# pratyushkumar211/industrial_nnmpc_2021

Measured on AMD Instinct MI355X. Metric: condensed-QP solves/sec (CDU offline datagen), higher is better.
Workload: dtype f64; 1 GPU; cdu_offline_data: synthetic CDU-size plant (n=4480 vars, m=8960 box rows, n_aug=284), 100000 sampled x0 per GPU per step, whole sequences u* written out; batch_per_gpu=100000, total_batch=100000, method=auto, parallelism=dp1 (sharded samples, 1 RCCL gather of the first moves pe...

## Files before the change

### include/nnmpc.h

```cpp
#ifndef NNMPC_H
#define NNMPC_H
#include <stdint.h>
#ifdef __cplusplus
extern "C" {
#endif

#define NNMPC_OK 0
#define NNMPC_EINVAL (-1)
#define NNMPC_EHIP (-2)
#define NNMPC_ENOMEM (-3)
#define NNMPC_ENOTIMPL (-4)

#define NNMPC_HOST 0
#define NNMPC_DEVICE 1

#define NNMPC_ST_OPTIMAL 0
#define NNMPC_ST_MAXITER 1
#define NNMPC_ST_NUMERIC 2

typedef struct nnmpc_qp nnmpc_qp;
typedef struct nnmpc_nn nnmpc_nn;

typedef struct {
  int32_t max_batch;
// ... 76 lines not shown
                            int32_t* status, int32_t* iters, int32_t ptr_kind, int32_t out_kind);

int nnmpc_qp_set_inverse(nnmpc_qp* h, const double* Hinv, const double* Kunc);

int nnmpc_qp_set_farfield(nnmpc_qp* h, int32_t W, int32_t r, const double* U, const double* Vx, const double* Vl);
int nnmpc_qp_farfield_missing(nnmpc_qp* h, int32_t* W);

int nnmpc_qp_first_moves(const double* u, int64_t ldu, const double* us, int32_t B, int32_t nu, double* out);
int nnmpc_qp_dims(nnmpc_qp* h, int32_t* n, int32_t* nu, int32_t* n_aug);
int nnmpc_qp_set_profiling(nnmpc_qp* h, int32_t on);
int nnmpc_qp_get_stats(nnmpc_qp* h, nnmpc_qp_stats* out, int32_t reset);

int nnmpc_qp_debug_factor_solve(nnmpc_qp* h, int32_t B, const float* dvec, const float* mask,
                                const float* rhs, float* sol);
int nnmpc_qp_debug_factor_fail(nnmpc_qp* h, int32_t B, int32_t* fail);

int nnmpc_nn_create(nnmpc_nn** out, int32_t nlayers, const int32_t* dims,
                    const double* const* W, const double* const* b, int32_t nx, int32_t nu,
                    int32_t with_uprev, const double* xscale, const double* ulb,
                    const double* uub, int32_t use_bf16, int32_t max_batch);
#define NNMPC_NN_STRUCTURED 0
#define NNMPC_NN_UNSTD 1
#define NNMPC_NN_UNSTD_RELU 2
int nnmpc_nn_create_ex(nnmpc_nn** out, int32_t nlayers, const int32_t* dims,
                       const double* const* W, const double* const* b, int32_t nx, int32_t nu,
                       int32_t with_uprev, const double* xscale, const double* ulb,
                       const double* uub, int32_t use_bf16, int32_t max_batch, int32_t form);
int nnmpc_nn_destroy(nnmpc_nn* h);
int nnmpc_nn_forward(nnmpc_nn* h, int32_t B, const double* x, const double* uprev,
                     const double* xs, const double* us, double* u, int32_t ptr_kind);
// ... 136 lines not shown
```

### industrial_nnmpc_2021_amd/_lib.py

```python
import ctypes as C
import os

_HERE = os.path.dirname(os.path.abspath(__file__))
LIB_PATH = os.path.join(_HERE, "libnnmpc_hip.so")

HOST, DEVICE = 0, 1
ST_OPTIMAL, ST_MAXITER, ST_NUMERIC = 0, 1, 2
OUT_SEQUENCE, OUT_FIRST_MOVE = 0, 1
EINVAL, EHIP, ENOMEM, ENOTIMPL = -1, -2, -3, -4


class QpOpts(C.Structure):
    _fields_ = [("max_batch", C.c_int32), ("nb", C.c_int32), ("max_ipm_iters", C.c_int32),
                ("max_polish_rounds", C.c_int32), ("max_refine", C.c_int32),
                ("max_rounds", C.c_int32), ("sub_steps", C.c_int32), ("stale_max_changes", C.c_int32),
                ("stale_cg_limit", C.c_int32), ("method", C.c_int32), ("asm_max_active", C.c_int32),
                ("asm_max_rounds", C.c_int32), ("asm_f32_rounds", C.c_int32), ("seg_max", C.c_int32), ("asm_tail_batch", C.c_int32), ("asm_predict_iters", C.c_int32), ("asm_overlap", C.c_int32), ("ipm_tol", C.c_float), ("refine_tol", C.c_double),
                ("bound_tol", C.c_double)]


class QpStats(C.Structure):
    _fields_ = [("problems", C.c_int64), ("rounds", C.c_int64), ("factorizations", C.c_int64),
                ("ipm_iterations", C.c_int64), ("panel_launches", C.c_int64),
                ("panel_ms", C.c_double), ("diag_ms", C.c_double), ("trsv_ms", C.c_double),
# ... 16 lines not shown
class ClModel(C.Structure):
    _fields_ = [(k, C.c_int32) for k in ("nx", "nu", "ny", "nd", "nz")] + \
               [(k, C.c_void_p) for k in ("A", "B", "C", "Bp", "Aaug", "Baug", "Caug", "L", "tb", "Qb", "Qy", "q0", "Cd",
                                          "Eb", "Xb", "Xu", "Qaug", "Raug", "Maug", "ulb", "uub", "x0", "xhat0", "uprev0")]


class ClSlot(C.Structure):
    _fields_ = [("kind", C.c_int32), ("qp", C.c_void_p), ("nlayers", C.c_int32), ("dims", C.c_void_p), ("W", C.c_void_p),
                ("b", C.c_void_p), ("with_uprev", C.c_int32), ("xscale", C.c_void_p), ("Kaug", C.c_void_p)]


EXPORTS = ["nnmpc_last_error", "nnmpc_qp_create", "nnmpc_qp_destroy", "nnmpc_qp_solve_batch",
           "nnmpc_qp_solve_batch_warm", "nnmpc_qp_solve_batch_ex", "nnmpc_qp_set_inverse", "nnmpc_qp_dims",
           "nnmpc_qp_first_moves", "nnmpc_qp_set_farfield", "nnmpc_qp_farfield_missing",
           "nnmpc_qp_set_profiling", "nnmpc_qp_get_stats", "nnmpc_qp_debug_factor_solve", "nnmpc_qp_debug_factor_fail",
           "nnmpc_nn_create", "nnmpc_nn_create_ex", "nnmpc_nn_destroy", "nnmpc_nn_forward", "nnmpc_nn_last_ms", "nnmpc_nn_last_hidden_ms",
           "nnmpc_train_create", "nnmpc_train_destroy", "nnmpc_train_set_data", "nnmpc_train_grad", "nnmpc_train_step",
           "nnmpc_train_epoch", "nnmpc_train_eval", "nnmpc_train_get_weights", "nnmpc_train_set_weights",
           "nnmpc_train_snapshot", "nnmpc_train_restore", "nnmpc_train_last_ms", "nnmpc_train_dw_slices",
           "nnmpc_train_padding_max",
           "nnmpc_train_group_create", "nnmpc_train_group_destroy", "nnmpc_train_group_set_data",
           "nnmpc_train_group_epoch", "nnmpc_train_group_eval", "nnmpc_train_group_get_weights",
           "nnmpc_train_group_set_weights", "nnmpc_train_group_snapshot", "nnmpc_train_group_restore",
           "nnmpc_train_group_padding_max", "nnmpc_train_group_last_ms", "nnmpc_train_group_last_launches",
           "nnmpc_chain_create", "nnmpc_chain_destroy", "nnmpc_chain_run", "nnmpc_chain_reset", "nnmpc_chain_last_ms",
           "nnmpc_ts_create", "nnmpc_ts_destroy", "nnmpc_ts_solve_batch",
           "nnmpc_cl_create", "nnmpc_cl_destroy", "nnmpc_cl_run", "nnmpc_cl_reset", "nnmpc_cl_last_ms",
           "nnmpc_cl_set_plant", "nnmpc_cl_last_plant_ms", "nnmpc_cstrs_flow",
           "nnmpc_device_count", "nnmpc_set_device", "nnmpc_device_synchronize", "nnmpc_dev_mem_info",
           "nnmpc_dev_malloc", "nnmpc_dev_free", "nnmpc_dev_memset", "nnmpc_memcpy_h2d", "nnmpc_memcpy_d2h",
# ... 30 lines not shown
    lib.nnmpc_qp_solve_batch_warm.argtypes = [vp, i32, dp, dp, dp, dp, dp, dp, dp, dp, i32]
    lib.nnmpc_qp_set_inverse.restype = i32
    lib.nnmpc_qp_set_inverse.argtypes = [vp, dp, dp]
    lib.nnmpc_qp_set_farfield.restype = i32
    lib.nnmpc_qp_set_farfield.argtypes = [vp, i32, i32, dp, dp, dp]
    lib.nnmpc_qp_farfield_missing.restype = i32
    lib.nnmpc_qp_farfield_missing.argtypes = [vp, C.POINTER(i32)]
    lib.nnmpc_qp_set_profiling.restype = i32
    lib.nnmpc_qp_set_profiling.argtypes = [vp, i32]
    lib.nnmpc_qp_get_stats.restype = i32
    lib.nnmpc_qp_get_stats.argtypes = [vp, C.POINTER(QpStats), i32]
    lib.nnmpc_qp_debug_factor_solve.restype = i32
    lib.nnmpc_qp_debug_factor_solve.argtypes = [vp, i32, dp, dp, dp, dp]
    lib.nnmpc_qp_debug_factor_fail.restype = i32
    lib.nnmpc_qp_debug_factor_fail.argtypes = [vp, i32, dp]
    lib.nnmpc_nn_create.restype = i32
    lib.nnmpc_nn_create.argtypes = [C.POINTER(vp), i32, C.POINTER(i32), C.POINTER(dp), C.POINTER(dp),
                                    i32, i32, i32, dp, dp, dp, i32, i32]
    lib.nnmpc_nn_create_ex.restype = i32
    lib.nnmpc_nn_create_ex.argtypes = lib.nnmpc_nn_create.argtypes + [i32]
    lib.nnmpc_nn_destroy.restype = i32
    lib.nnmpc_nn_destroy.argtypes = [vp]
    lib.nnmpc_nn_forward.restype = i32
    lib.nnmpc_nn_forward.argtypes = [vp, i32, dp, dp, dp, dp, dp, i32]
    lib.nnmpc_nn_last_ms.restype = i32
    lib.nnmpc_nn_last_ms.argtypes = [vp, C.POINTER(C.c_double), C.POINTER(C.c_double)]
    lib.nnmpc_nn_last_hidden_ms.restype = i32
    lib.nnmpc_nn_last_hidden_ms.argtypes = [vp, C.POINTER(C.c_double), C.POINTER(C.c_int32)]
    f64, pf64, pi32, pdp = C.c_double, C.POINTER(C.c_double), C.POINTER(i32), C.POINTER(dp)
    lib.nnmpc_train_create.restype = i32
# ... 196 lines not shown
```

### industrial_nnmpc_2021_amd/csrc/qp_predict.h

```cpp
#pragma once
#include "qp_asm.h"

namespace nnmpc {

typedef __bf16 pbf16x8 __attribute__((ext_vector_type(8)));
typedef float pf32x4 __attribute__((ext_vector_type(4)));
typedef unsigned int pu32x4 __attribute__((ext_vector_type(4)));
typedef unsigned int pu32x2 __attribute__((ext_vector_type(2)));
typedef float pf32x2 __attribute__((ext_vector_type(2)));
typedef __bf16 pbf16x2 __attribute__((ext_vector_type(2)));
typedef _Float16 pf16x2 __attribute__((ext_vector_type(2)));

constexpr int PRED_NW = 8;
constexpr int PRED_MAXIT = 64;
template <int NT> struct PredCfg {
  static constexpr int W = 16 * NT * PRED_NW;
  static constexpr int KS = W / 32;
  static constexpr int LDY = W + 8;
};
constexpr int PRED_W = PredCfg<4>::W;
constexpr int PRED_W2 = PredCfg<8>::W;

struct PredArgs {
  const pu32x4* Hf;
  int iters;
  int* itsum;
  int fac10;
  int adaptive;
  float beta[PRED_MAXIT];
};

template <int NT, int PT> __host__ __device__ constexpr int pred_lds_bytes(int nu) {
  return 16 * PT * PredCfg<NT>::LDY * 2 + 2 * 16 * PT * (nu + 4) * 4 + 16;
}

template <int NT> __host__ __device__ constexpr size_t pred_frag_index(int jtg, int ks, int lane) {
  return (((size_t)(jtg / NT) * PredCfg<NT>::KS + ks) * NT + (jtg % NT)) * 64 + lane;
}

__device__ __forceinline__ unsigned pred_bf16(float x) {
  const unsigned u = __float_as_uint(x);
  return (u + 0x7fffu + ((u >> 16) & 1u)) >> 16;
}

template <int NT, int PT, bool NU4 = true>
__global__ __launch_bounds__(64 * PRED_NW, 2) void asm_predict_k(AsmDev d, PredArgs a) {
  extern __shared__ __attribute__((aligned(16))) unsigned char sm_raw[];
  constexpr int KS = PredCfg<NT>::KS, LDY = PredCfg<NT>::LDY, MR = 16 * PT;
  unsigned short* Y = reinterpret_cast<unsigned short*>(sm_raw);
  const int ldb = d.nu + 4;
  float* lbs = reinterpret_cast<float*>(Y + MR * LDY);
  float* ubs = lbs + MR * ldb;
  int* nviol = reinterpret_cast<int*>(ubs + MR * ldb);
  float* rsum = reinterpret_cast<float*>(nviol + 1);
  constexpr int NTH = 64 * PRED_NW;
  const int tid = threadIdx.x, lane = tid & 63, w = __builtin_amdgcn_readfirstlane(tid >> 6);
  const int li = lane & 15, lq = lane >> 4;
  const int p0 = blockIdx.x * MR;
  for (int i = tid; i < MR * d.nu; i += NTH) {
    const int r = i / d.nu, k = i - r * d.nu;
    const size_t p = (size_t)min(p0 + r, d.nseg - 1);
    lbs[r * ldb + k] = (float)d.lb[p * d.nu + k];
    ubs[r * ldb + k] = (float)d.ub[p * d.nu + k];
  }
  for (int i = tid; i < MR * LDY / 2; i += NTH) reinterpret_cast<unsigned*>(Y)[i] = 0u;
  if (tid == 0) { *nviol = 0; rsum[0] = 0.f; rsum[1] = 0.f; }
  unsigned sx[NT][PT][2], sm[NT][PT][2];
#pragma unroll
  for (int jt = 0; jt < NT; ++jt)
#pragma unroll
    for (int pt = 0; pt < PT; ++pt) {
      const size_t p = (size_t)min(p0 + 16 * pt + li, d.nseg - 1);
      const double* xr = d.xunc + p * d.np + 16 * (w * NT + jt) + 4 * lq;
#pragma unroll
      for (int h = 0; h < 2; ++h) {
        const pf32x2 xu = {fminf(fmaxf((float)xr[2 * h], -60000.f), 60000.f), fminf(fmaxf((float)xr[2 * h + 1], -60000.f), 60000.f)};
        sx[jt][pt][h] = __builtin_bit_cast(unsigned, __builtin_convertvector(xu, pf16x2));
        sm[jt][pt][h] = 0u;
      }
    }
  int kc0[NT];
#pragma unroll
  for (int jt = 0; jt < NT; ++jt) kc0[jt] = (16 * (w * NT + jt) + 4 * lq) % d.nu;
  const bool st_words = (d.n & 3) == 0;
  const bool per32 = 32 % d.nu == 0;
  __syncthreads();
  const __amdgpu_buffer_rsrc_t rH = __builtin_amdgcn_make_buffer_rsrc(const_cast<pu32x4*>(a.Hf), 0, PRED_NW * KS * NT * 1024, 0x00020000);
  const int l16 = lane * 16;
  const int hw0 = w * (KS * NT * 1024);
  auto hload = [&](int ksn, int jt) __attribute__((always_inline)) {
    return __builtin_bit_cast(pu32x4, __builtin_amdgcn_raw_buffer_load_b128(rH, l16 + jt * 1024, hw0 + ksn * (NT * 1024), 0));
  };
  int nit = a.iters;
  int kb = 0;
  for (int it = 0; it < nit; ++it) {
    if (tid == 0) rsum[it & 1] = 0.f;
    pf32x4 acc[NT][PT];
#pragma unroll
    for (int jt = 0; jt < NT; ++jt)
#pragma unroll
      for (int pt = 0; pt < PT; ++pt) acc[jt][pt] = pf32x4{0.f, 0.f, 0.f, 0.f};
#ifdef PRED_NO_MFMA
    if (false) {
#else
    if (it > 0) {
#endif
      constexpr int RD = 3;
      pu32x4 hb[RD][NT];
      asm_sfor<0, RD - 1>([&](auto bc) __attribute__((always_inline)) {
        constexpr int b = decltype(bc)::value;
#pragma unroll
        for (int jt = 0; jt < NT; ++jt) hb[b][jt] = hload(b, jt);
      });
      asm_sfor<0, KS>([&](auto kc) __attribute__((always_inline)) {
        constexpr int ks = decltype(kc)::value, b = ks % RD;
        if constexpr (ks + RD - 1 < KS) {
#pragma unroll
          for (int jt = 0; jt < NT; ++jt) hb[(ks + RD - 1) % RD][jt] = hload(ks + RD - 1, jt);
        }
        pu32x4 yf[PT];
#pragma unroll
        for (int pt = 0; pt < PT; ++pt) yf[pt] = *reinterpret_cast<const pu32x4*>(Y + (16 * pt + li) * LDY + 32 * ks + 8 * lq);
#pragma unroll
        for (int jt = 0; jt < NT; ++jt)
#pragma unroll
          for (int pt = 0; pt < PT; ++pt)
            acc[jt][pt] = __builtin_amdgcn_mfma_f32_16x16x32_bf16(__builtin_bit_cast(pbf16x8, hb[b][jt]), __builtin_bit_cast(pbf16x8, yf[pt]),
                                                                  acc[jt][pt], 0, 0, 0);
        __builtin_amdgcn_sched_barrier(0);
      });
    }
    __syncthreads();
    if (it > 0) kb = rsum[(it - 1) & 1] > 0.f ? 0 : kb + 1;
    const pf32x2 beta2 = {a.beta[kb], a.beta[kb]};
    pf32x2 rdot = {0.f, 0.f};
    int yo = li * LDY + 16 * NT * w + 4 * lq, bo = li * ldb;
    asm volatile("" : "+v"(yo), "+v"(bo));
    unsigned short* Yl = Y + yo;
    const float* lbl = lbs + bo;
    const float* ubl = ubs + bo;
    int nv0 = 0;
#pragma unroll
    for (int pt = 0; pt < PT; ++pt) {
      pf32x4 lb4[2], ub4[2];
#pragma unroll
      for (int jt = 0; jt < NT; ++jt) {
        if constexpr (NU4) {
          if (jt < 2 || !per32) {
            lb4[jt & 1] = *reinterpret_cast<const pf32x4*>(lbl + 16 * pt * ldb + kc0[jt]);
            ub4[jt & 1] = *reinterpret_cast<const pf32x4*>(ubl + 16 * pt * ldb + kc0[jt]);
          }
        } else {
#pragma unroll
          for (int r = 0; r < 4; ++r) {
            const int k = kc0[jt] + r, kk = k >= d.nu ? k - d.nu : k;
            lb4[jt & 1][r] = lbl[16 * pt * ldb + kk];
            ub4[jt & 1][r] = ubl[16 * pt * ldb + kk];
          }
        }
        unsigned short* yp = Yl + 16 * pt * LDY + 16 * jt;
        const pu32x2 yw = *reinterpret_cast<const pu32x2*>(yp);
        unsigned yb[2];
#pragma unroll
        for (int h = 0; h < 2; ++h) {
          const pf32x2 xu = __builtin_convertvector(__builtin_bit_cast(pf16x2, sx[jt][pt][h]), pf32x2);
          const unsigned mw = sm[jt][pt][h], ywd = yw[h];
          const pf32x2 nu = {__uint_as_float(mw << 16), __uint_as_float(mw & 0xffff0000u)};
          const pf32x2 y = {__uint_as_float(ywd << 16), __uint_as_float(ywd & 0xffff0000u)};
          const pf32x2 ac = {acc[jt][pt][2 * h], acc[jt][pt][2 * h + 1]};
#ifdef PRED_NO_EPI
          const pf32x2 wv = xu - ac;
#else
          const pf32x2 wv = y + (xu - ac);
#endif
          const pf32x2 cl = {__builtin_amdgcn_fmed3f(wv[0], lb4[jt & 1][2 * h], ub4[jt & 1][2 * h]),
                             __builtin_amdgcn_fmed3f(wv[1], lb4[jt & 1][2 * h + 1], ub4[jt & 1][2 * h + 1])};
          const pf32x2 nun = wv - cl;
          const pf32x2 dn = nun - nu;
          const pf32x2 yn = beta2 * dn + nun;
          rdot += (y - nun) * dn;
// ... 69 lines not shown
```

### industrial_nnmpc_2021_amd/csrc/qp_solver.hip

```cpp
#include <hip/hip_runtime.h>
#include <stdint.h>
#include <stdio.h>
#include <stdarg.h>
#include <string.h>
#include <vector>
#include <algorithm>
#include <cmath>
#include <cstdlib>
#include "../../include/nnmpc.h"
#define ASM_WG_TU (-1)
#include "chol_kernels.h"
#include "gemm_kernels.h"
#include "qp_asm.h"
#include "qp_wide.h"
#include "qp_small.h"
#include "qp_predict.h"
#include "common.h"
static constexpr int ASM_SMALL9_LDS_MAX = 100 * 1024;

using namespace nnmpc;

namespace {

enum { PH_INIT = 0, PH_IPM = 1, PH_POLISH = 2, PH_DONE = 3 };
// ... 613 lines not shown
  struct Far { int W, r, rp; double *U, *Vx, *Vl, *cu; int* kt; double ksum; double efar; };
  std::vector<Far> far;
  std::vector<int> far_missing;
  double p_inf = 0.0;
  double *asm_tnorm = nullptr, *asm_tslack = nullptr;
  struct AsmView {
    double *lam = nullptr, *xh = nullptr, *xhw = nullptr, *tnorm = nullptr, *tslack = nullptr;
    float *lam32 = nullptr, *xh32 = nullptr;
    int *rowprob = nullptr, *kblk = nullptr, *counters = nullptr;
    int rows = 0;
  };
  AsmView view[2];
  struct PredWin { pu32x4* Hf = nullptr; double L = 0.0; int W = 0; };
  PredWin pred[2];
  int* pred_cnt = nullptr;
  double* asm_work;
  int seg_max;
  double* x0_64;
  float* x0_32;
  double* q64_all;
  float* uunc_all;
  double *lb_d, *ub_d;
  double* in_stage;
  hipStream_t stream;
  hipStream_t stream2 = nullptr;
  hipStream_t stream3 = nullptr, stream4 = nullptr;
  int asm_tail_budget = 50000;
  hipEvent_t ev_fork = nullptr, ev_join = nullptr, ev_join3 = nullptr, ev_join4 = nullptr;
  hipEvent_t ev_wfork = nullptr, ev_wide = nullptr;
  int* pin_cnt = nullptr;
// ... 329 lines not shown
        if (force_w >= 0) wide = force_w;
        else {
          HIPCHK(hipMemsetAsync(h->pred_cnt, 0, 4, s));
          hipLaunchKernelGGL(asm_extent_k, dim3((nprob + 63) / 64), dim3(256), 0, s, a, PRED_W - PRED_W / 4, PRED_W, h->pred_cnt);
          HIPCHK(hipMemcpyAsync(h->pin_cnt, h->pred_cnt, 4, hipMemcpyDeviceToHost, s));
          HIPCHK(stream_sync(s));
          wide = h->pin_cnt[0] * 4 > nprob;
          h->pin_cnt[0] = 0;
        }
      }
      if (wide && Wx < PRED_W2) {
        EvScope es(h, 5, 2.0 * (PRED_W2 - Wx) * (double)h->ka * nprob);
        gemm64(h, h->asm_xunc + Wx, h->np, h->x0_64, h->ka, h->Kunc64 + (size_t)Wx * h->ka, h->ka, segp, PRED_W2 - Wx, h->ka);
        Wx = PRED_W2; a.Wx = Wx;
      }
      const bool nu4 = h->nu % 4 == 0;
      const int W = wide ? PRED_W2 : PRED_W, MR = (wide || !nu4) ? 32 : 64;
      pa.Hf = h->pred[wide].Hf;
      pred_flops_per_it = 2.0 * W * (double)W * MR;
      h->stats.asm_predict_launches += 1;
      EvScope es(h, 10, 0.0);
      if (wide) hipLaunchKernelGGL((asm_predict_k<8, 2>), dim3((nprob + 31) / 32), dim3(64 * PRED_NW), (pred_lds_bytes<8, 2>(h->nu)), s, a, pa);
      else if (nu4) hipLaunchKernelGGL((asm_predict_k<4, 4>), dim3((nprob + 63) / 64), dim3(64 * PRED_NW), (pred_lds_bytes<4, 4>(h->nu)), s, a, pa);
      else hipLaunchKernelGGL((asm_predict_k<4, 2, false>), dim3((nprob + 31) / 32), dim3(64 * PRED_NW), (pred_lds_bytes<4, 2>(h->nu)), s, a, pa);
      a.pred_w = W;
      { static const int pf = getenv("NNMPC_PRED_F64") ? atoi(getenv("NNMPC_PRED_F64")) : 0; a.pred_f64 = pf; }
    }
  }
  hipLaunchKernelGGL(asm_init_k, dim3((segp + 3) / 4), dim3(256), 0, s, a, segp);
  const int lds_big = (a.max_active + ASM_TS) * 8;
  int* cnt = h->pin_cnt;
  memset(cnt, 0, 2 * ASM_NCNT * sizeof(int));
  int rounds = 0;
  int kprev = 0;
  HIPCHK(hipMemsetAsync(h->asm_counters, 0, 2 * ASM_NCNT * sizeof(int), s));
  if (small) {
    EvScope es(h, 4, 0.0);
    static const int g0 = getenv("NNMPC_SMALL_GRACE") ? atoi(getenv("NNMPC_SMALL_GRACE")) : ASM_SM_GRACE;
    hipLaunchKernelGGL((asm_small_k<2, 3, 4>), dim3(nprob), dim3(64), asm_small_lds_bytes(2, h->n, h->nu), s, a, a.max_rounds, g0);
    hipLaunchKernelGGL((asm_small_k<7, 1, 8>), dim3(nprob), dim3(64), asm_small_lds_bytes(7, h->n, h->nu), s, a, a.max_rounds, g0);
// ... 601 lines not shown
}

int nnmpc_qp_destroy(nnmpc_qp* h) {
  if (!h) return NNMPC_OK;
  hipDeviceSynchronize();
  for (void* p : h->allocs) hipFree(p);
  for (auto& g : h->far) { hipFree(g.U); hipFree(g.Vx); hipFree(g.Vl); hipFree(g.cu); hipFree(g.kt); }
  for (auto& sc : h->sc) if (sc.p) hipFree(sc.p);
  for (hipEvent_t e : h->ev_pool) hipEventDestroy(e);
  if (h->ev_fork) hipEventDestroy(h->ev_fork);
  if (h->ev_join) hipEventDestroy(h->ev_join);
  if (h->ev_join3) hipEventDestroy(h->ev_join3);
  if (h->ev_join4) hipEventDestroy(h->ev_join4);
  if (h->ev_wfork) hipEventDestroy(h->ev_wfork);
  if (h->ev_wide) hipEventDestroy(h->ev_wide);
  if (h->pin_cnt) hipHostFree(h->pin_cnt);
  if (h->pin_st) hipHostFree(h->pin_st);
  if (h->stream2) hipStreamDestroy(h->stream2);
  if (h->stream3) hipStreamDestroy(h->stream3);
  if (h->stream4) hipStreamDestroy(h->stream4);
  if (h->stream) hipStreamDestroy(h->stream);
  delete h;
  return NNMPC_OK;
}

int nnmpc_qp_set_inverse(nnmpc_qp* h, const double* Hinv, const double* Kunc) {
  if (!h || !Hinv || !Kunc) { set_error("nnmpc_qp_set_inverse: bad arguments"); return NNMPC_EINVAL; }
  HIPCHK(hipSetDevice(h->device));
  const int n = h->n, np = h->np, ka = h->ka, n_aug = h->n_aug;
  if ((uint64_t)np * np * 8 >= (1ull << 32)) {
// ... 6 lines not shown
    for (int k = 0; k < n_aug; ++k) kk[(size_t)r * ka + k] = Kunc[(size_t)r * n_aug + k];
  }
  HIPCHK(hipMemcpy(h->H64, hh.data(), hh.size() * 8, hipMemcpyHostToDevice));
  {
    std::vector<float> h32(hh.size());
    for (size_t i = 0; i < hh.size(); ++i) h32[i] = (float)hh[i];
    HIPCHK(hipMemcpy(h->H32, h32.data(), h32.size() * 4, hipMemcpyHostToDevice));
  }
  HIPCHK(hipMemcpy(h->Kunc64, kk.data(), kk.size() * 8, hipMemcpyHostToDevice));
  h->pred[0].L = h->pred[1].L = 0.0;
  if (h->nu <= 64 && h->nu >= 4 && h->opts.asm_predict_iters >= 0) {
    if (np >= PRED_W && n >= PRED_W) {
      const int rc = build_predictor<4>(h, hh, np, h->pred[0]);
      if (rc) return rc;
      if (!h->pred_cnt) { const int rc2 = dev_alloc(h, &h->pred_cnt, 4); if (rc2) return rc2; }
      HIPCHK(hipFuncSetAttribute((const void*)asm_predict_k<4, 4>, hipFuncAttributeMaxDynamicSharedMemorySize, pred_lds_bytes<4, 4>(h->nu)));
      HIPCHK(hipFuncSetAttribute((const void*)asm_predict_k<4, 2, false>, hipFuncAttributeMaxDynamicSharedMemorySize, pred_lds_bytes<4, 2>(h->nu)));
    }
    if (np >= PRED_W2 && n >= PRED_W2 && h->pred[0].L > 0.0 && h->nu % 4 == 0) {
      const int rc = build_predictor<8>(h, hh, np, h->pred[1]);
      if (rc) return rc;
      HIPCHK(hipFuncSetAttribute((const void*)asm_predict_k<8, 2>, hipFuncAttributeMaxDynamicSharedMemorySize, pred_lds_bytes<8, 2>(h->nu)));
    }
  }
  {
    const int kap = ((n_aug + 63) / 64) * 64;
    double *tmp = nullptr, *kt = nullptr;
    const size_t ntmp = (size_t)np * std::max(np, kap);
    HIPCHK(hipMalloc((void**)&tmp, ntmp * 8));
    HIPCHK(hipMalloc((void**)&kt, (size_t)kap * np * 8));
    std::vector<double> ktr((size_t)kap * np, 0.0);
    for (int r = 0; r < n; ++r)
// ... 114 lines not shown

int nnmpc_qp_dims(nnmpc_qp* h, int32_t* n, int32_t* nu, int32_t* n_aug) {
  if (!h) { set_error("nnmpc_qp_dims: null handle"); return NNMPC_EINVAL; }
  if (n) *n = h->n;
  if (nu) *nu = h->nu;
  if (n_aug) *n_aug = h->n_aug;
  return NNMPC_OK;
}

int nnmpc_qp_set_profiling(nnmpc_qp* h, int32_t on) {
  if (!h) return NNMPC_EINVAL;
  h->profiling = on != 0;
  return NNMPC_OK;
}

int nnmpc_qp_get_stats(nnmpc_qp* h, nnmpc_qp_stats* out, int32_t reset) {
  if (!h || !out) return NNMPC_EINVAL;
  *out = h->stats;
  out->asm_e1max = h->asm_e1max; out->asm_e2max = h->asm_e2max;
  {
    std::vector<double> w(3 * (size_t)h->seg_max, 0.0);
    hipMemcpy(w.data(), h->asm_work, w.size() * sizeof(double), hipMemcpyDeviceToHost);
    double f = 0.0, b = 0.0, f32 = 0.0;
    for (size_t i = 0; i < w.size(); i += 3) { f += w[i]; b += w[i + 1]; f32 += w[i + 2]; }
    out->asm_lambda_flops = f; out->asm_lambda_bytes = b; out->asm_lambda32_flops = f32;
    if (reset) hipMemset(h->asm_work, 0, w.size() * sizeof(double));
  }
  {
    unsigned long long c = 0;
    hipMemcpy(&c, h->trsv_count, sizeof(c), hipMemcpyDeviceToHost);
// ... 26 lines not shown
  const int ncol = out_kind == NNMPC_OUT_FIRST_MOVE ? h->nu : h->n;
  h->ldu = ncol; h->nout = ncol;
  size_t e_tot0 = 0;
  if (h->profiling) { e_tot0 = ev_get(h); hipEventRecord(h->ev_pool[e_tot0], h->stream); }
  double* u_stage = nullptr; uint32_t* a_stage = nullptr; int32_t* s_stage = nullptr; int32_t* i_stage = nullptr;
  unsigned char* g_stage = nullptr;
  const int gmax = std::min(G, (int)B);
  int rc = 0;
  if (ptr_kind == NNMPC_HOST) {
    if (!rc) rc = scratch_get(h, nnmpc_qp::SC_U, &u_stage, (size_t)gmax * ncol * sizeof(double));
    if (!rc && active) rc = scratch_get(h, nnmpc_qp::SC_ACT, &a_stage, (size_t)gmax * h->words * sizeof(uint32_t));
    if (!rc && status) rc = scratch_get(h, nnmpc_qp::SC_ST, &s_stage, (size_t)gmax * sizeof(int32_t));
    if (!rc && iters) rc = scratch_get(h, nnmpc_qp::SC_IT, &i_stage, (size_t)gmax * 2 * sizeof(int32_t));
    if (!rc && guess) rc = scratch_get(h, nnmpc_qp::SC_GUESS, &g_stage, (size_t)gmax * h->n);
  }
  hipError_t he = hipSuccess;
#define STEP_(x) do { if (!rc && he == hipSuccess) { he = (x); if (he != hipSuccess) { set_error("%s: %s", #x, hipGetErrorString(he)); rc = NNMPC_EHIP; } } } while (0)
  for (int b0 = 0; b0 < B && !rc; b0 += G) {
    const int nb = std::min(G, B - b0);
    const double *x0d, *lbd, *ubd;
    double* ud; uint32_t* ad; int32_t* sd; int32_t* idv;
    const unsigned char* gd = nullptr;
    if (ptr_kind == NNMPC_HOST) {
      if (guess) { STEP_(hipMemcpyAsync(g_stage, guess + (size_t)b0 * h->n, (size_t)nb * h->n, hipMemcpyHostToDevice, h->stream)); gd = g_stage; }
      STEP_(hipMemcpyAsync(h->in_stage, x0 + (size_t)b0 * h->n_aug, (size_t)nb * h->n_aug * 8, hipMemcpyHostToDevice, h->stream));
      STEP_(hipMemcpyAsync(h->lb_d, lb + (size_t)b0 * h->nu, (size_t)nb * h->nu * 8, hipMemcpyHostToDevice, h->stream));
      STEP_(hipMemcpyAsync(h->ub_d, ub + (size_t)b0 * h->nu, (size_t)nb * h->nu * 8, hipMemcpyHostToDevice, h->stream));
      x0d = h->in_stage; lbd = h->lb_d; ubd = h->ub_d;
      ud = u_stage; ad = active ? a_stage : nullptr; sd = status ? s_stage : nullptr; idv = iters ? i_stage : nullptr;
    } else {
      x0d = x0 + (size_t)b0 * h->n_aug; lbd = lb + (size_t)b0 * h->nu; ubd = ub + (size_t)b0 * h->nu;
      if (guess) gd = guess + (size_t)b0 * h->n;
      ud = u + (size_t)b0 * ncol;
      ad = active ? active + (size_t)b0 * h->words : nullptr;
      sd = status ? status + b0 : nullptr;
      idv = iters ? iters + 2 * (size_t)b0 : nullptr;
    }
    if (rc) break;
    if (h->have_inverse && h->opts.method != 1) rc = solve_segment_asm(h, nb, x0d, lbd, ubd, gd, ud, ad, sd, idv);
    else rc = solve_segment(h, nb, x0d, lbd, ubd, gd, ud, ad, sd, idv);
    if (!rc && ptr_kind == NNMPC_HOST) {
      STEP_(hipMemcpy(u + (size_t)b0 * ncol, u_stage, (size_t)nb * ncol * 8, hipMemcpyDeviceToHost));
      if (active) STEP_(hipMemcpy(active + (size_t)b0 * h->words, a_stage, (size_t)nb * h->words * 4, hipMemcpyDeviceToHost));
      if (status) STEP_(hipMemcpy(status + b0, s_stage, (size_t)nb * 4, hipMemcpyDeviceToHost));
      if (iters) STEP_(hipMemcpy(iters + 2 * (size_t)b0, i_stage, (size_t)nb * 8, hipMemcpyDeviceToHost));
    }
  }
#undef STEP_
  if (h->profiling) {
    size_t e1 = ev_get(h);
    hipEventRecord(h->ev_pool[e1], h->stream);
    stream_sync(h->stream);
    h->ev_recs.push_back({3, e_tot0, e1, 0.0});
// ... 48 lines not shown
```

### industrial_nnmpc_2021_amd/qp.py

```python
import ctypes as C
import numpy as np

from . import _lib


def _ptr(a):
    if a is None:
        return None, None
    if hasattr(a, "data_ptr"):
        return C.c_void_p(a.data_ptr()), _lib.DEVICE
    return a.ctypes.data_as(C.c_void_p), _lib.HOST


def _staircase(U0, tol, block=128, chunk=16):
    import scipy.linalg as sla
    nf, r = U0.shape
    nb = -(-nf // block)
    Rs = [None] * nb
    below = np.zeros((0, r))
    for j in range(nb - 1, -1, -1):
        below = Rs[j] = sla.qr(np.vstack((U0[j * block:(j + 1) * block], below)), mode="r")[0][:r]
    cur = np.eye(r)
    drops, kj = [], np.zeros(nb, int)
    for j in range(nb):
# ... 7 lines not shown
        kj[j] = cur.shape[0]
    G = np.vstack([cur] + drops[:0:-1])
    if G.shape[0] == 0:
        G = np.eye(1, r)
    kj = np.minimum(-(-kj // chunk) * chunk, G.shape[0])
    U1 = U0 @ G.T
    for j in range(nb):
        U1[j * block:(j + 1) * block, kj[j]:] = 0.0
    return np.ascontiguousarray(U1), G


class BatchedBoxQP:

    def __init__(self, P, tq, nu, *, Kunc="auto", method="auto", farfield="auto", max_batch=1024, nb=0, ipm_tol=0.0,
                 max_rounds=0, max_ipm_iters=0, max_polish_rounds=0, max_refine=0, sub_steps=0, stale_max_changes=0, stale_cg_limit=0, asm_max_active=0,
                 asm_max_rounds=0, asm_f32_rounds=0, seg_max=0, asm_tail_batch=0, asm_predict_iters=0, asm_overlap=0):
        lib = _lib.load()
        P = np.ascontiguousarray(P, dtype=np.float64)
        tq = np.ascontiguousarray(tq, dtype=np.float64)
        n, n_aug = tq.shape
        if P.shape != (n, n) or n % nu:
            raise ValueError("P must be (n, n), tq (n, n_aug), n a multiple of nu")
        meth = {"auto": 0, "pdip": 1, "asm": 2}[method]
        Hinv = None
        if isinstance(Kunc, str) and Kunc == "auto":
            import scipy.linalg as sla
            Ps = np.tril(P) + np.tril(P, -1).T
            cf = sla.cho_factor(Ps, lower=True)
            Kunc = -sla.cho_solve(cf, tq)
            if meth != 1:
                Hinv = sla.cho_solve(cf, np.eye(n))
# ... 4 lines not shown
        self.n, self.n_aug, self.nu = n, n_aug, nu
        self.words = (2 * n + 31) // 32
        opts = _lib.QpOpts(max_batch=max_batch, nb=nb, max_ipm_iters=max_ipm_iters,
                           max_polish_rounds=max_polish_rounds, max_refine=max_refine,
                           max_rounds=max_rounds, sub_steps=sub_steps, stale_max_changes=stale_max_changes,
                           stale_cg_limit=stale_cg_limit, method=meth, asm_max_active=asm_max_active,
                           asm_max_rounds=asm_max_rounds, asm_f32_rounds=asm_f32_rounds, seg_max=seg_max, asm_tail_batch=asm_tail_batch,
                           asm_predict_iters=asm_predict_iters, asm_overlap=asm_overlap,
                           ipm_tol=ipm_tol, refine_tol=0.0, bound_tol=0.0)
        self._h = C.c_void_p()
        kp = Kunc.ctypes.data_as(C.c_void_p) if Kunc is not None else None
        _lib.check(lib.nnmpc_qp_create(C.byref(self._h), n, nu, n_aug,
                                       P.ctypes.data_as(C.c_void_p), tq.ctypes.data_as(C.c_void_p),
                                       kp, C.byref(opts)), "nnmpc_qp_create")
        self._lib = lib
        self.have_inverse = False
        if Hinv is not None:
            Hinv = np.ascontiguousarray(Hinv, dtype=np.float64)
            rc = lib.nnmpc_qp_set_inverse(self._h, Hinv.ctypes.data_as(C.c_void_p), Kunc.ctypes.data_as(C.c_void_p))
            if rc == _lib.EINVAL and meth == 0:
                import warnings
                warnings.warn("BatchedBoxQP: " + lib.nnmpc_last_error().decode(errors="replace") +
                              " -- continuing with the PDIP path only", RuntimeWarning)
            else:
                _lib.check(rc, "nnmpc_qp_set_inverse")
                self.have_inverse = True
        self._ff_wmax = (n // 2 // 128) * 128
        self._ff_src = (np.ascontiguousarray(Hinv[:, :self._ff_wmax]), Kunc) if (self.have_inverse and farfield and self._ff_wmax > 0) else None
        nb_lib = nb if nb else (128 if n > 1024 else 64)
        self._np = -(-n // nb_lib) * nb_lib
# ... 88 lines not shown
                           first_move_only=False):
        q = lambda a: (_ptr(a)[0] if a is not None else None)
        _lib.check(self._lib.nnmpc_qp_solve_batch_ex(
            self._h, B, q(x0), q(lb), q(ub), q(guess), q(u), q(active), q(status), q(iters), _lib.DEVICE,
            _lib.OUT_FIRST_MOVE if first_move_only else _lib.OUT_SEQUENCE), "nnmpc_qp_solve_batch_ex")
        self._farfield_auto()

    def set_profiling(self, on=True):
        _lib.check(self._lib.nnmpc_qp_set_profiling(self._h, int(on)), "nnmpc_qp_set_profiling")

    def stats(self, reset=False):
        s = _lib.QpStats()
        _lib.check(self._lib.nnmpc_qp_get_stats(self._h, C.byref(s), int(reset)), "nnmpc_qp_get_stats")
        return {k: getattr(s, k) for k, _ in s._fields_}

    def debug_factor_solve(self, dvec, mask, rhs):
        dvec = np.ascontiguousarray(dvec, np.float32)
        mask = np.ascontiguousarray(mask, np.float32)
        rhs = np.ascontiguousarray(rhs, np.float32)
        B = dvec.shape[0]
        sol = np.empty((B, self.n), np.float32)
        _lib.check(self._lib.nnmpc_qp_debug_factor_solve(
            self._h, B, *(a.ctypes.data_as(C.c_void_p) for a in (dvec, mask, rhs, sol))),
            "nnmpc_qp_debug_factor_solve")
        return sol

    def debug_factor_fail(self, B):
        fail = np.empty(B, np.int32)
        _lib.check(self._lib.nnmpc_qp_debug_factor_fail(self._h, B, fail.ctypes.data_as(C.c_void_p)),
                   "nnmpc_qp_debug_factor_fail")
# ... 2 lines not shown
```

Baseline: 7.612 million solves/s.

## Swizzle predictor LDS layout, stage x in LDS, and hoist H prefetch

```diff
diff --git a/include/nnmpc.h b/include/nnmpc.h
--- a/include/nnmpc.h
+++ b/include/nnmpc.h
@@ -114,6 +114,8 @@
 int nnmpc_qp_debug_factor_solve(nnmpc_qp* h, int32_t B, const float* dvec, const float* mask,
                                 const float* rhs, float* sol);
 int nnmpc_qp_debug_factor_fail(nnmpc_qp* h, int32_t B, int32_t* fail);
+int nnmpc_qp_debug_keep_predicted(nnmpc_qp* h, int32_t on);
+int nnmpc_qp_debug_predicted(nnmpc_qp* h, int32_t B, uint8_t* st, int32_t* rows, int32_t* W, double* L);
 
 int nnmpc_nn_create(nnmpc_nn** out, int32_t nlayers, const int32_t* dims,
                     const double* const* W, const double* const* b, int32_t nx, int32_t nu,
diff --git a/industrial_nnmpc_2021_amd/_lib.py b/industrial_nnmpc_2021_amd/_lib.py
--- a/industrial_nnmpc_2021_amd/_lib.py
+++ b/industrial_nnmpc_2021_amd/_lib.py
@@ -54,6 +54,7 @@
            "nnmpc_qp_solve_batch_warm", "nnmpc_qp_solve_batch_ex", "nnmpc_qp_set_inverse", "nnmpc_qp_dims",
            "nnmpc_qp_first_moves", "nnmpc_qp_set_farfield", "nnmpc_qp_farfield_missing",
            "nnmpc_qp_set_profiling", "nnmpc_qp_get_stats", "nnmpc_qp_debug_factor_solve", "nnmpc_qp_debug_factor_fail",
+           "nnmpc_qp_debug_keep_predicted", "nnmpc_qp_debug_predicted",
            "nnmpc_nn_create", "nnmpc_nn_create_ex", "nnmpc_nn_destroy", "nnmpc_nn_forward", "nnmpc_nn_last_ms", "nnmpc_nn_last_hidden_ms",
            "nnmpc_train_create", "nnmpc_train_destroy", "nnmpc_train_set_data", "nnmpc_train_grad", "nnmpc_train_step",
            "nnmpc_train_epoch", "nnmpc_train_eval", "nnmpc_train_get_weights", "nnmpc_train_set_weights",
@@ -114,6 +115,10 @@
     lib.nnmpc_qp_debug_factor_solve.argtypes = [vp, i32, dp, dp, dp, dp]
     lib.nnmpc_qp_debug_factor_fail.restype = i32
     lib.nnmpc_qp_debug_factor_fail.argtypes = [vp, i32, dp]
+    lib.nnmpc_qp_debug_keep_predicted.restype = i32
+    lib.nnmpc_qp_debug_keep_predicted.argtypes = [vp, i32]
+    lib.nnmpc_qp_debug_predicted.restype = i32
+    lib.nnmpc_qp_debug_predicted.argtypes = [vp, i32, dp, C.POINTER(i32), C.POINTER(i32), C.POINTER(C.c_double)]
     lib.nnmpc_nn_create.restype = i32
     lib.nnmpc_nn_create.argtypes = [C.POINTER(vp), i32, C.POINTER(i32), C.POINTER(dp), C.POINTER(dp),
                                     i32, i32, i32, dp, dp, dp, i32, i32]
diff --git a/industrial_nnmpc_2021_amd/csrc/qp_predict.h b/industrial_nnmpc_2021_amd/csrc/qp_predict.h
--- a/industrial_nnmpc_2021_amd/csrc/qp_predict.h
+++ b/industrial_nnmpc_2021_amd/csrc/qp_predict.h
@@ -16,10 +16,10 @@
 template <int NT> struct PredCfg {
   static constexpr int W = 16 * NT * PRED_NW;
   static constexpr int KS = W / 32;
-  static constexpr int LDY = W + 8;
 };
 constexpr int PRED_W = PredCfg<4>::W;
 constexpr int PRED_W2 = PredCfg<8>::W;
+constexpr int PRED_LDS_MAX = 160 * 1024;
 
 struct PredArgs {
   const pu32x4* Hf;
@@ -30,8 +30,25 @@
   float beta[PRED_MAXIT];
 };
 
-template <int NT, int PT> __host__ __device__ constexpr int pred_lds_bytes(int nu) {
-  return 16 * PT * PredCfg<NT>::LDY * 2 + 2 * 16 * PT * (nu + 4) * 4 + 16;
+template <int NT> __host__ __device__ constexpr int pred_y_index(int row, int col) {
+  return row * PredCfg<NT>::W + ((((col >> 3) ^ (row & 15)) << 3) | (col & 7));
+}
+template <int NT> __host__ __device__ constexpr int pred_y_frag(int fb, int fc, int ks, int pt) {
+  return 16 * pt * PredCfg<NT>::W + fb + ((32 * ks) ^ fc);
+}
+template <int NT> __host__ __device__ constexpr int pred_y_epi(int yb, int yc, int jt, int pt) {
+  return 16 * pt * PredCfg<NT>::W + yb + ((16 * jt) ^ yc);
+}
+__host__ __device__ constexpr int pred_bnd_ld(int nu, bool nu4 = true) { return (nu4 && (nu == 32 || nu == 16 || nu == 8 || nu == 4)) ? nu : nu + 4; }
+__host__ __device__ constexpr int pred_bnd_index(int row, int k, int nu, bool nu4 = true) {
+  int slot = k >> 2;
+  if (nu4 && nu == 32) slot ^= (row >> 1) & 7;
+  else if (nu4 && nu == 16) slot ^= (0 - (row >> 2)) & 3;
+  return row * pred_bnd_ld(nu, nu4) + 4 * slot + (k & 3);
+}
+
+template <int NT, int PT, bool NU4 = true> __host__ __device__ constexpr int pred_lds_bytes(int nu) {
+  return 2 * 16 * PT * PredCfg<NT>::W * 2 + 2 * 16 * PT * pred_bnd_ld(nu, NU4) * 4 + 16;
 }
 
 template <int NT> __host__ __device__ constexpr size_t pred_frag_index(int jtg, int ks, int lane) {
@@ -46,10 +63,11 @@
 template <int NT, int PT, bool NU4 = true>
 __global__ __launch_bounds__(64 * PRED_NW, 2) void asm_predict_k(AsmDev d, PredArgs a) {
   extern __shared__ __attribute__((aligned(16))) unsigned char sm_raw[];
-  constexpr int KS = PredCfg<NT>::KS, LDY = PredCfg<NT>::LDY, MR = 16 * PT;
+  constexpr int KS = PredCfg<NT>::KS, W = PredCfg<NT>::W, MR = 16 * PT;
   unsigned short* Y = reinterpret_cast<unsigned short*>(sm_raw);
-  const int ldb = d.nu + 4;
-  float* lbs = reinterpret_cast<float*>(Y + MR * LDY);
+  unsigned short* X = Y + MR * W;
+  const int ldb = pred_bnd_ld(d.nu, NU4);
+  float* lbs = reinterpret_cast<float*>(X + MR * W);
   float* ubs = lbs + MR * ldb;
   int* nviol = reinterpret_cast<int*>(ubs + MR * ldb);
   float* rsum = reinterpret_cast<float*>(nviol + 1);
@@ -60,28 +78,40 @@
   for (int i = tid; i < MR * d.nu; i += NTH) {
     const int r = i / d.nu, k = i - r * d.nu;
     const size_t p = (size_t)min(p0 + r, d.nseg - 1);
-    lbs[r * ldb + k] = (float)d.lb[p * d.nu + k];
-    ubs[r * ldb + k] = (float)d.ub[p * d.nu + k];
-  }
-  for (int i = tid; i < MR * LDY / 2; i += NTH) reinterpret_cast<unsigned*>(Y)[i] = 0u;
+    lbs[pred_bnd_index(r, k, d.nu, NU4)] = (float)d.lb[p * d.nu + k];
+    ubs[pred_bnd_index(r, k, d.nu, NU4)] = (float)d.ub[p * d.nu + k];
+  }
+  for (int i = tid; i < MR * W / 2; i += NTH) reinterpret_cast<unsigned*>(Y)[i] = 0u;
   if (tid == 0) { *nviol = 0; rsum[0] = 0.f; rsum[1] = 0.f; }
-  unsigned sx[NT][PT][2], sm[NT][PT][2];
+  const int yb0 = li * W + 4 * (lq & 1), yc0 = 8 * ((2 * w * NT) ^ (lq >> 1) ^ li);
+  int kc0[NT];
+#pragma unroll
+  for (int jt = 0; jt < NT; ++jt) {
+    const int k0 = (16 * (w * NT + jt) + 4 * lq) % d.nu;
+    kc0[jt] = pred_bnd_index(li, k0, d.nu, NU4) - li * ldb;
+  }
+  unsigned sm[NT][PT][2];
+#ifdef PRED_X_REGS
+  unsigned sx[NT][PT][2];
+#endif
 #pragma unroll
   for (int jt = 0; jt < NT; ++jt)
 #pragma unroll
     for (int pt = 0; pt < PT; ++pt) {
       const size_t p = (size_t)min(p0 + 16 * pt + li, d.nseg - 1);
       const double* xr = d.xunc + p * d.np + 16 * (w * NT + jt) + 4 * lq;
+      unsigned xw[2];
 #pragma unroll
       for (int h = 0; h < 2; ++h) {
         const pf32x2 xu = {fminf(fmaxf((float)xr[2 * h], -60000.f), 60000.f), fminf(fmaxf((float)xr[2 * h + 1], -60000.f), 60000.f)};
-        sx[jt][pt][h] = __builtin_bit_cast(unsigned, __builtin_convertvector(xu, pf16x2));
+        xw[h] = __builtin_bit_cast(unsigned, __builtin_convertvector(xu, pf16x2));
         sm[jt][pt][h] = 0u;
+#ifdef PRED_X_REGS
+        sx[jt][pt][h] = xw[h];
+#endif
       }
-    }
-  int kc0[NT];
-#pragma unroll
-  for (int jt = 0; jt < NT; ++jt) kc0[jt] = (16 * (w * NT + jt) + 4 * lq) % d.nu;
+      *reinterpret_cast<pu32x2*>(X + pred_y_epi<NT>(yb0, yc0, jt, pt)) = pu32x2{xw[0], xw[1]};
+    }
   const bool st_words = (d.n & 3) == 0;
   const bool per32 = 32 % d.nu == 0;
   __syncthreads();
@@ -89,10 +119,19 @@
   const int l16 = lane * 16;
   const int hw0 = w * (KS * NT * 1024);
   auto hload = [&](int ksn, int jt) __attribute__((always_inline)) {
-    return __builtin_bit_cast(pu32x4, __builtin_amdgcn_raw_buffer_load_b128(rH, l16 + jt * 1024, hw0 + ksn * (NT * 1024), 0));
+    return __builtin_bit_cast(pu32x4, __builtin_amdgcn_raw_buffer_load_b128(rH, l16 + (jt & 3) * 1024, hw0 + ksn * (NT * 1024) + (jt >> 2) * 4096, 0));
   };
   int nit = a.iters;
   int kb = 0;
+  constexpr int RD = 3;
+  pu32x4 hb[RD][NT];
+  auto hfirst = [&]() __attribute__((always_inline)) {
+    asm_sfor<0, RD - 1>([&](auto bc) __attribute__((always_inline)) {
+      constexpr int b = decltype(bc)::value;
+#pragma unroll
+      for (int jt = 0; jt < NT; ++jt) hb[b][jt] = hload(b, jt);
+    });
+  };
   for (int it = 0; it < nit; ++it) {
     if (tid == 0) rsum[it & 1] = 0.f;
     pf32x4 acc[NT][PT];
@@ -105,27 +144,39 @@
 #else
     if (it > 0) {
 #endif
-      constexpr int RD = 3;
-      pu32x4 hb[RD][NT];
-      asm_sfor<0, RD - 1>([&](auto bc) __attribute__((always_inline)) {
-        constexpr int b = decltype(bc)::value;
-#pragma unroll
-        for (int jt = 0; jt < NT; ++jt) hb[b][jt] = hload(b, jt);
-      });
+      int lh = l16;
+      asm volatile("" : "+v"(lh));
+      const int fb = ((lh >> 4) & 15) * W, fc = 8 * (((lh >> 4) & 15) ^ (lh >> 8));
+#ifndef PRED_H_AHEAD
+      hfirst();
+#endif
+#ifdef PRED_Y_AHEAD
+      pu32x4 yf[2][PT];
+#pragma unroll
+      for (int pt = 0; pt < PT; ++pt) yf[0][pt] = *reinterpret_cast<const pu32x4*>(Y + pred_y_frag<NT>(fb, fc, 0, pt));
+#endif
       asm_sfor<0, KS>([&](auto kc) __attribute__((always_inline)) {
         constexpr int ks = decltype(kc)::value, b = ks % RD;
         if constexpr (ks + RD - 1 < KS) {
 #pragma unroll
           for (int jt = 0; jt < NT; ++jt) hb[(ks + RD - 1) % RD][jt] = hload(ks + RD - 1, jt);
         }
-        pu32x4 yf[PT];
-#pragma unroll
-        for (int pt = 0; pt < PT; ++pt) yf[pt] = *reinterpret_cast<const pu32x4*>(Y + (16 * pt + li) * LDY + 32 * ks + 8 * lq);
+#ifdef PRED_Y_AHEAD
+        if constexpr (ks + 1 < KS) {
+#pragma unroll
+          for (int pt = 0; pt < PT; ++pt) yf[(ks + 1) & 1][pt] = *reinterpret_cast<const pu32x4*>(Y + pred_y_frag<NT>(fb, fc, ks + 1, pt));
+        }
+        const pu32x4* yk = yf[ks & 1];
+#else
+        pu32x4 yk[PT];
+#pragma unroll
+        for (int pt = 0; pt < PT; ++pt) yk[pt] = *reinterpret_cast<const pu32x4*>(Y + pred_y_frag<NT>(fb, fc, ks, pt));
+#endif
 #pragma unroll
         for (int jt = 0; jt < NT; ++jt)
 #pragma unroll
           for (int pt = 0; pt < PT; ++pt)
-            acc[jt][pt] = __builtin_amdgcn_mfma_f32_16x16x32_bf16(__builtin_bit_cast(pbf16x8, hb[b][jt]), __builtin_bit_cast(pbf16x8, yf[pt]),
+            acc[jt][pt] = __builtin_amdgcn_mfma_f32_16x16x32_bf16(__builtin_bit_cast(pbf16x8, hb[b][jt]), __builtin_bit_cast(pbf16x8, yk[pt]),
                                                                   acc[jt][pt], 0, 0, 0);
         __builtin_amdgcn_sched_barrier(0);
       });
@@ -134,14 +185,16 @@
     if (it > 0) kb = rsum[(it - 1) & 1] > 0.f ? 0 : kb + 1;
     const pf32x2 beta2 = {a.beta[kb], a.beta[kb]};
     pf32x2 rdot = {0.f, 0.f};
-    int yo = li * LDY + 16 * NT * w + 4 * lq, bo = li * ldb;
-    asm volatile("" : "+v"(yo), "+v"(bo));
-    unsigned short* Yl = Y + yo;
+    int yb = yb0, yc = yc0, bo = li * ldb;
+    asm volatile("" : "+v"(yb), "+v"(yc), "+v"(bo));
     const float* lbl = lbs + bo;
     const float* ubl = ubs + bo;
     int nv0 = 0;
 #pragma unroll
     for (int pt = 0; pt < PT; ++pt) {
+#ifdef PRED_H_AHEAD
+      if (pt == PT - 1) hfirst();
+#endif
       pf32x4 lb4[2], ub4[2];
 #pragma unroll
       for (int jt = 0; jt < NT; ++jt) {
@@ -158,12 +211,17 @@
             ub4[jt & 1][r] = ubl[16 * pt * ldb + kk];
           }
         }
-        unsigned short* yp = Yl + 16 * pt * LDY + 16 * jt;
+        unsigned short* yp = Y + pred_y_epi<NT>(yb, yc, jt, pt);
         const pu32x2 yw = *reinterpret_cast<const pu32x2*>(yp);
+#ifdef PRED_X_REGS
+        const pu32x2 xw = {sx[jt][pt][0], sx[jt][pt][1]};
+#else
+        const pu32x2 xw = *reinterpret_cast<const pu32x2*>(X + pred_y_epi<NT>(yb, yc, jt, pt));
+#endif
         unsigned yb[2];
 #pragma unroll
         for (int h = 0; h < 2; ++h) {
-          const pf32x2 xu = __builtin_convertvector(__builtin_bit_cast(pf16x2, sx[jt][pt][h]), pf32x2);
+          const pf32x2 xu = __builtin_convertvector(__builtin_bit_cast(pf16x2, xw[h]), pf32x2);
           const unsigned mw = sm[jt][pt][h], ywd = yw[h];
           const pf32x2 nu = {__uint_as_float(mw << 16), __uint_as_float(mw & 0xffff0000u)};
           const pf32x2 y = {__uint_as_float(ywd << 16), __uint_as_float(ywd & 0xffff0000u)};
diff --git a/industrial_nnmpc_2021_amd/csrc/qp_solver.hip b/industrial_nnmpc_2021_amd/csrc/qp_solver.hip
--- a/industrial_nnmpc_2021_amd/csrc/qp_solver.hip
+++ b/industrial_nnmpc_2021_amd/csrc/qp_solver.hip
@@ -651,6 +651,11 @@
   struct PredWin { pu32x4* Hf = nullptr; double L = 0.0; int W = 0; };
   PredWin pred[2];
   int* pred_cnt = nullptr;
+  bool keep_pred = false;
+  unsigned char* pred_keep = nullptr;
+  size_t pred_keep_cap = 0;
+  int pred_keep_rows = 0, pred_keep_w = 0, seg_b0 = 0;
+  double pred_keep_L = 0.0;
   double* asm_work;
   int seg_max;
   double* x0_64;
@@ -1010,7 +1015,7 @@
         gemm64(h, h->asm_xunc + Wx, h->np, h->x0_64, h->ka, h->Kunc64 + (size_t)Wx * h->ka, h->ka, segp, PRED_W2 - Wx, h->ka);
         Wx = PRED_W2; a.Wx = Wx;
       }
-      const bool nu4 = h->nu % 4 == 0;
+      const bool nu4 = h->nu % 4 == 0 && pred_lds_bytes<4, 4>(h->nu) <= PRED_LDS_MAX;
       const int W = wide ? PRED_W2 : PRED_W, MR = (wide || !nu4) ? 32 : 64;
       pa.Hf = h->pred[wide].Hf;
       pred_flops_per_it = 2.0 * W * (double)W * MR;
@@ -1018,8 +1023,14 @@
       EvScope es(h, 10, 0.0);
       if (wide) hipLaunchKernelGGL((asm_predict_k<8, 2>), dim3((nprob + 31) / 32), dim3(64 * PRED_NW), (pred_lds_bytes<8, 2>(h->nu)), s, a, pa);
       else if (nu4) hipLaunchKernelGGL((asm_predict_k<4, 4>), dim3((nprob + 63) / 64), dim3(64 * PRED_NW), (pred_lds_bytes<4, 4>(h->nu)), s, a, pa);
-      else hipLaunchKernelGGL((asm_predict_k<4, 2, false>), dim3((nprob + 31) / 32), dim3(64 * PRED_NW), (pred_lds_bytes<4, 2>(h->nu)), s, a, pa);
+      else hipLaunchKernelGGL((asm_predict_k<4, 2, false>), dim3((nprob + 31) / 32), dim3(64 * PRED_NW), (pred_lds_bytes<4, 2, false>(h->nu)), s, a, pa);
       a.pred_w = W;
+      if (h->keep_pred && h->pred_keep) {
+        if (h->pred_keep_w == 0 || h->pred_keep_w == W) {
+          HIPCHK(hipMemcpy2DAsync(h->pred_keep + (size_t)h->seg_b0 * W, W, a.st, h->n, W, nprob, hipMemcpyDeviceToDevice, s));
+          h->pred_keep_w = W; h->pred_keep_rows = h->seg_b0 + nprob; h->pred_keep_L = h->pred[wide].L;
+        } else h->pred_keep_w = -1;
+      }
       { static const int pf = getenv("NNMPC_PRED_F64") ? atoi(getenv("NNMPC_PRED_F64")) : 0; a.pred_f64 = pf; }
     }
   }
@@ -1651,6 +1662,7 @@
   if (h->ev_join4) hipEventDestroy(h->ev_join4);
   if (h->ev_wfork) hipEventDestroy(h->ev_wfork);
   if (h->ev_wide) hipEventDestroy(h->ev_wide);
+  if (h->pred_keep) hipFree(h->pred_keep);
   if (h->pin_cnt) hipHostFree(h->pin_cnt);
   if (h->pin_st) hipHostFree(h->pin_st);
   if (h->stream2) hipStreamDestroy(h->stream2);
@@ -1687,8 +1699,9 @@
       const int rc = build_predictor<4>(h, hh, np, h->pred[0]);
       if (rc) return rc;
       if (!h->pred_cnt) { const int rc2 = dev_alloc(h, &h->pred_cnt, 4); if (rc2) return rc2; }
-      HIPCHK(hipFuncSetAttribute((const void*)asm_predict_k<4, 4>, hipFuncAttributeMaxDynamicSharedMemorySize, pred_lds_bytes<4, 4>(h->nu)));
-      HIPCHK(hipFuncSetAttribute((const void*)asm_predict_k<4, 2, false>, hipFuncAttributeMaxDynamicSharedMemorySize, pred_lds_bytes<4, 2>(h->nu)));
+      if (h->nu % 4 == 0 && pred_lds_bytes<4, 4>(h->nu) <= PRED_LDS_MAX)
+        HIPCHK(hipFuncSetAttribute((const void*)asm_predict_k<4, 4>, hipFuncAttributeMaxDynamicSharedMemorySize, pred_lds_bytes<4, 4>(h->nu)));
+      HIPCHK(hipFuncSetAttribute((const void*)asm_predict_k<4, 2, false>, hipFuncAttributeMaxDynamicSharedMemorySize, pred_lds_bytes<4, 2, false>(h->nu)));
     }
     if (np >= PRED_W2 && n >= PRED_W2 && h->pred[0].L > 0.0 && h->nu % 4 == 0) {
       const int rc = build_predictor<8>(h, hh, np, h->pred[1]);
@@ -1833,6 +1846,27 @@
   return NNMPC_OK;
 }
 
+int nnmpc_qp_debug_keep_predicted(nnmpc_qp* h, int32_t on) {
+  if (!h) return NNMPC_EINVAL;
+  h->keep_pred = on != 0;
+  if (!h->keep_pred) { h->pred_keep_rows = 0; h->pred_keep_w = 0; }
+  return NNMPC_OK;
+}
+
+int nnmpc_qp_debug_predicted(nnmpc_qp* h, int32_t B, uint8_t* st, int32_t* rows, int32_t* W, double* L) {
+  if (!h || B < 0) { set_error("nnmpc_qp_debug_predicted: bad arguments"); return NNMPC_EINVAL; }
+  const bool have = h->keep_pred && h->pred_keep && h->pred_keep_w > 0;
+  if (rows) *rows = have ? h->pred_keep_rows : 0;
+  if (W) *W = have ? h->pred_keep_w : 0;
+  if (L) *L = have ? h->pred_keep_L : 0.0;
+  if (!st || !have) return NNMPC_OK;
+  if (B > h->pred_keep_rows) { set_error("nnmpc_qp_debug_predicted: %d rows asked for, %d kept", B, h->pred_keep_rows); return NNMPC_EINVAL; }
+  HIPCHK(hipSetDevice(h->device));
+  HIPCHK(stream_sync(h->stream));
+  HIPCHK(hipMemcpy(st, h->pred_keep, (size_t)B * h->pred_keep_w, hipMemcpyDeviceToHost));
+  return NNMPC_OK;
+}
+
 int nnmpc_qp_get_stats(nnmpc_qp* h, nnmpc_qp_stats* out, int32_t reset) {
   if (!h || !out) return NNMPC_EINVAL;
   *out = h->stats;
@@ -1889,6 +1923,16 @@
     if (!rc && iters) rc = scratch_get(h, nnmpc_qp::SC_IT, &i_stage, (size_t)gmax * 2 * sizeof(int32_t));
     if (!rc && guess) rc = scratch_get(h, nnmpc_qp::SC_GUESS, &g_stage, (size_t)gmax * h->n);
   }
+  if (h->keep_pred) {
+    h->pred_keep_rows = 0; h->pred_keep_w = 0;
+    const size_t need = (size_t)B * PRED_W2;
+    if (need > h->pred_keep_cap) {
+      if (h->pred_keep) hipFree(h->pred_keep);
+      h->pred_keep = nullptr; h->pred_keep_cap = 0;
+      if (hipMalloc((void**)&h->pred_keep, need) != hipSuccess) { set_error("nnmpc_qp_solve_batch: no memory for the copy of the predicted states"); return NNMPC_ENOMEM; }
+      h->pred_keep_cap = need;
+    }
+  }
   hipError_t he = hipSuccess;
 #define STEP_(x) do { if (!rc && he == hipSuccess) { he = (x); if (he != hipSuccess) { set_error("%s: %s", #x, hipGetErrorString(he)); rc = NNMPC_EHIP; } } } while (0)
   for (int b0 = 0; b0 < B && !rc; b0 += G) {
@@ -1912,6 +1956,7 @@
       idv = iters ? iters + 2 * (size_t)b0 : nullptr;
     }
     if (rc) break;
+    h->seg_b0 = b0;
     if (h->have_inverse && h->opts.method != 1) rc = solve_segment_asm(h, nb, x0d, lbd, ubd, gd, ud, ad, sd, idv);
     else rc = solve_segment(h, nb, x0d, lbd, ubd, gd, ud, ad, sd, idv);
     if (!rc && ptr_kind == NNMPC_HOST) {
diff --git a/industrial_nnmpc_2021_amd/qp.py b/industrial_nnmpc_2021_amd/qp.py
--- a/industrial_nnmpc_2021_amd/qp.py
+++ b/industrial_nnmpc_2021_amd/qp.py
@@ -45,7 +45,7 @@
 
     def __init__(self, P, tq, nu, *, Kunc="auto", method="auto", farfield="auto", max_batch=1024, nb=0, ipm_tol=0.0,
                  max_rounds=0, max_ipm_iters=0, max_polish_rounds=0, max_refine=0, sub_steps=0, stale_max_changes=0, stale_cg_limit=0, asm_max_active=0,
-                 asm_max_rounds=0, asm_f32_rounds=0, seg_max=0, asm_tail_batch=0, asm_predict_iters=0, asm_overlap=0):
+                 asm_max_rounds=0, asm_f32_rounds=0, seg_max=0, asm_tail_batch=0, asm_predict_iters=0, asm_overlap=0, keep_predicted=False):
         lib = _lib.load()
         P = np.ascontiguousarray(P, dtype=np.float64)
         tq = np.ascontiguousarray(tq, dtype=np.float64)
@@ -80,6 +80,8 @@
                                        P.ctypes.data_as(C.c_void_p), tq.ctypes.data_as(C.c_void_p),
                                        kp, C.byref(opts)), "nnmpc_qp_create")
         self._lib = lib
+        if keep_predicted:
+            _lib.check(lib.nnmpc_qp_debug_keep_predicted(self._h, 1), "nnmpc_qp_debug_keep_predicted")
         self.have_inverse = False
         if Hinv is not None:
             Hinv = np.ascontiguousarray(Hinv, dtype=np.float64)
@@ -198,6 +200,16 @@
         _lib.check(self._lib.nnmpc_qp_get_stats(self._h, C.byref(s), int(reset)), "nnmpc_qp_get_stats")
         return {k: getattr(s, k) for k, _ in s._fields_}
 
+    def predicted_states(self):
+        rows, W, L = C.c_int32(0), C.c_int32(0), C.c_double(0.0)
+        _lib.check(self._lib.nnmpc_qp_debug_predicted(self._h, 0, None, C.byref(rows), C.byref(W), C.byref(L)), "nnmpc_qp_debug_predicted")
+        if W.value <= 0 or rows.value <= 0:
+            return None
+        st = np.empty((rows.value, W.value), np.uint8)
+        _lib.check(self._lib.nnmpc_qp_debug_predicted(self._h, rows.value, st.ctypes.data_as(C.c_void_p), None, None, None),
+                   "nnmpc_qp_debug_predicted")
+        return dict(states=st, W=int(W.value), L=float(L.value))
+
     def debug_factor_solve(self, dvec, mask, rhs):
         dvec = np.ascontiguousarray(dvec, np.float32)
         mask = np.ascontiguousarray(mask, np.float32)
```

After: 3.467 million solves/s. 0.456x the previous value.
